# microsoft/rl-offline-simulation

Measured on AMD Instinct MI355X. Metric: simulated steps/sec (node), 10M logged transitions x 4096 rollouts, higher is better.
Workload: dtype f64

## Files before the change

### rl-offline-simulation_amd/csrc/offsim_hip.hip

```cpp
#include <hip/hip_fp16.h>
#include <hip/hip_runtime.h>
#include <mutex>
#include <stdint.h>
#include <stdio.h>
#include <stdlib.h>
#include <string.h>
#include <time.h>

#include "offsim.h"
#include "discount.hpp"
#include "pcg64_dev.hpp"
#include "philox_dev.hpp"
#include "stream_row.hpp"

extern "C" int offsim_lds_order_ok(void);
#include "shuffle_wave.hpp"
#include "shuffle_chunk.hpp"

using namespace offsim;

static thread_local char g_err[512] = "";

static int fail(int code, const char *fmt, const char *detail = "") {
    snprintf(g_err, sizeof(g_err), fmt, detail);
    return code;
}
#define HIP_TRY(expr)                                                        \
    do {                                                                     \
        hipError_t _e = (expr);                                              \
        if (_e != hipSuccess) return fail(OFFSIM_EHIP, #expr ": %s", hipGetErrorString(_e)); \
    } while (0)
#define LAUNCH_CHECK()                                                       \
    do {                                                                     \
        hipError_t _e = hipGetLastError();                                   \
        if (_e != hipSuccess) return fail(OFFSIM_EHIP, "kernel launch: %s", hipGetErrorString(_e)); \
    } while (0)

extern "C" const char *offsim_last_error(void) { return g_err; }
extern "C" int offsim_version(void) { return 100; }
extern "C" int offsim_device_count(void) {
    int n = 0;
    hipError_t e = hipGetDeviceCount(&n);
    if (e != hipSuccess) return fail(OFFSIM_EHIP, "hipGetDeviceCount: %s", hipGetErrorString(e));
    return n;
}


#define GRP_CHUNK 2048

__global__ void k_group_hist(const int32_t *__restrict__ slot, int64_t N, int32_t n_slots, uint32_t *__restrict__ hist) {
    extern __shared__ uint32_t lds_cnt[];
    for (int s = threadIdx.x; s < n_slots; s += blockDim.x) lds_cnt[s] = 0;
    __syncthreads();
    int64_t base = (int64_t)blockIdx.x * GRP_CHUNK;
    for (int i = threadIdx.x; i < GRP_CHUNK; i += blockDim.x) {
        int64_t row = base + i;
        if (row < N) atomicAdd(&lds_cnt[slot[row]], 1u);
    }
    __syncthreads();
    uint32_t *h = hist + (int64_t)blockIdx.x * n_slots;
    for (int s = threadIdx.x; s < n_slots; s += blockDim.x) h[s] = lds_cnt[s];
}

__global__ void k_group_scan_chunks(uint32_t *__restrict__ hist, int64_t n_chunks, int32_t n_slots, uint32_t *__restrict__ totals) {
    int s = blockIdx.x * blockDim.x + threadIdx.x;
    if (s >= n_slots) return;
    uint32_t run = 0;
    for (int64_t c = 0; c < n_chunks; c++) {
        uint32_t v = hist[c * n_slots + s];
        hist[c * n_slots + s] = run;
        run += v;
    }
    totals[s] = run;
}
__global__ void k_group_scan_slots(const uint32_t *__restrict__ totals, int32_t n_slots, uint32_t *__restrict__ seg_off) {
    uint32_t carry = 0;
    int lane = threadIdx.x;
    for (int b = 0; b < n_slots; b += WAVE) {
        int s = b + lane;
        uint32_t v = s < n_slots ? totals[s] : 0u;
        uint32_t inc = v;
#pragma unroll
        for (int d = 1; d < WAVE; d <<= 1) {
            uint32_t o = __shfl_up(inc, d);
            if (lane >= d) inc += o;
        }
        if (s < n_slots) seg_off[s] = carry + inc - v;
        carry += __shfl(inc, WAVE - 1);
    }
    if (lane == 0) seg_off[n_slots] = carry;
}
__global__ void k_group_scatter(const int32_t *__restrict__ slot, int64_t N, int32_t n_slots,
                                const uint32_t *__restrict__ hist, const uint32_t *__restrict__ seg_off,
                                int32_t *__restrict__ order) {
    extern __shared__ uint32_t lds_pos_raw[];
    volatile uint32_t *lds_pos = lds_pos_raw;
    const uint32_t *h = hist + (int64_t)blockIdx.x * n_slots;
    for (int s = threadIdx.x; s < n_slots; s += WAVE) lds_pos[s] = seg_off[s] + h[s];
    __syncthreads();
    int lane = threadIdx.x;
    int64_t base = (int64_t)blockIdx.x * GRP_CHUNK;
    for (int i = 0; i < GRP_CHUNK; i += WAVE) {
        int64_t row = base + i + lane;
        bool valid = row < N;
        int32_t key = valid ? slot[row] : -1;
        uint64_t todo = __ballot(valid);
        uint32_t dst = 0;
        while (todo) {
            int leader = __ffsll((unsigned long long)todo) - 1;
            int32_t k = __shfl(key, leader);
            uint64_t same = __ballot(valid && key == k);
            if (valid && key == k) {
                uint32_t before = __popcll(same & ((1ull << lane) - 1ull));
                dst = lds_pos[k] + before;
            }
            __builtin_amdgcn_s_waitcnt(0xc07f);
            if (lane == leader) lds_pos[k] += __popcll(same);
            todo &= ~same;
        }
        if (valid) order[dst] = (int32_t)row;
    }
}

extern "C" int64_t offsim_group_scratch_bytes(int64_t N, int32_t n_slots) {
    int64_t n_chunks = (N + GRP_CHUNK - 1) / GRP_CHUNK;
    if (n_chunks < 1) n_chunks = 1;
    return (n_chunks * n_slots + n_slots) * (int64_t)sizeof(uint32_t) + 256;
}

extern "C" int offsim_group_by_state(const int32_t *slot, int64_t N, int32_t n_slots, uint32_t *seg_off, int32_t *order,
                                     void *scratch, void *stream) {
    if (N < 0 || n_slots <= 0 || !seg_off || !scratch) return fail(OFFSIM_EINVAL, "group_by_state: bad argument%s");
    if ((int64_t)n_slots * 4 > 64 * 1024) return fail(OFFSIM_EUNSUPPORTED, "group_by_state: more than 16384 states%s");
    if (N >= (1ll << 31)) return fail(OFFSIM_EUNSUPPORTED, "group_by_state: N >= 2^31%s");
    hipStream_t st = (hipStream_t)stream;
    int64_t n_chunks = (N + GRP_CHUNK - 1) / GRP_CHUNK;
    uint32_t *hist = (uint32_t *)scratch;
    uint32_t *totals = hist + (n_chunks > 0 ? n_chunks : 1) * n_slots;
    if (n_chunks == 0) {
        HIP_TRY(hipMemsetAsync(seg_off, 0, sizeof(uint32_t) * (n_slots + 1), st));
        return OFFSIM_OK;
    }
    size_t lds = sizeof(uint32_t) * n_slots;
    hipLaunchKernelGGL(k_group_hist, dim3((unsigned)n_chunks), dim3(256), lds, st, slot, N, n_slots, hist);
    LAUNCH_CHECK();
    hipLaunchKernelGGL(k_group_scan_chunks, dim3((n_slots + 63) / 64), dim3(64), 0, st, hist, n_chunks, n_slots, totals);
    LAUNCH_CHECK();
    hipLaunchKernelGGL(k_group_scan_slots, dim3(1), dim3(WAVE), 0, st, totals, n_slots, seg_off);
    LAUNCH_CHECK();
    hipLaunchKernelGGL(k_group_scatter, dim3((unsigned)n_chunks), dim3(WAVE), lds, st, slot, N, n_slots, hist, seg_off, order);
    LAUNCH_CHECK();
    return OFFSIM_OK;
}

template <typename T>
__global__ void k_gather_elem(const T *__restrict__ src, const int32_t *__restrict__ order, int64_t N, T *__restrict__ dst) {
    int64_t g = (int64_t)blockIdx.x * blockDim.x + threadIdx.x;
    if (g < N) dst[g] = src[order[g]];
}
template <typename W>
__global__ void k_gather_words(const W *__restrict__ src, const int32_t *__restrict__ order, int64_t N, int32_t words, W *__restrict__ dst) {
    int64_t i = (int64_t)blockIdx.x * blockDim.x + threadIdx.x;
    if (i >= N * words) return;
    int64_t g = i / words;
    int32_t w = (int32_t)(i - g * words);
    dst[i] = src[(int64_t)order[g] * words + w];
}
extern "C" int offsim_gather_rows(const void *src, const int32_t *order, int64_t N, int32_t row_bytes, void *dst, void *stream) {
    if (N < 0 || row_bytes <= 0) return fail(OFFSIM_EINVAL, "gather_rows: bad argument%s");
    if (N == 0) return OFFSIM_OK;
    hipStream_t st = (hipStream_t)stream;
    unsigned nb = (unsigned)((N + 255) / 256);
    if (row_bytes == 1) hipLaunchKernelGGL(k_gather_elem<uint8_t>, dim3(nb), dim3(256), 0, st, (const uint8_t *)src, order, N, (uint8_t *)dst);
    else if (row_bytes == 2) hipLaunchKernelGGL(k_gather_elem<uint16_t>, dim3(nb), dim3(256), 0, st, (const uint16_t *)src, order, N, (uint16_t *)dst);
    else if (row_bytes == 4) hipLaunchKernelGGL(k_gather_elem<uint32_t>, dim3(nb), dim3(256), 0, st, (const uint32_t *)src, order, N, (uint32_t *)dst);
    else if (row_bytes == 8) hipLaunchKernelGGL(k_gather_elem<uint64_t>, dim3(nb), dim3(256), 0, st, (const uint64_t *)src, order, N, (uint64_t *)dst);
    else {
        const int32_t wb = row_bytes % 4 == 0 ? 4 : row_bytes % 2 == 0 ? 2 : 1, words = row_bytes / wb;
        unsigned nbw = (unsigned)((N * words + 255) / 256);
        if (wb == 4) hipLaunchKernelGGL(k_gather_words<uint32_t>, dim3(nbw), dim3(256), 0, st, (const uint32_t *)src, order, N, words, (uint32_t *)dst);
        else if (wb == 2) hipLaunchKernelGGL(k_gather_words<uint16_t>, dim3(nbw), dim3(256), 0, st, (const uint16_t *)src, order, N, words, (uint16_t *)dst);
        else hipLaunchKernelGGL(k_gather_words<uint8_t>, dim3(nbw), dim3(256), 0, st, (const uint8_t *)src, order, N, words, (uint8_t *)dst);
    }
    LAUNCH_CHECK();
    return OFFSIM_OK;
}

__global__ void k_seed_streams(const uint64_t *__restrict__ seeds, int32_t R, uint64_t *__restrict__ out) {
    int r = blockIdx.x * blockDim.x + threadIdx.x;
    if (r >= R) return;
    PcgInit p = pcg_seed(seeds[r]);
    out[4 * r + 0] = p.state.hi;
    out[4 * r + 1] = p.state.lo;
    out[4 * r + 2] = p.inc.hi;
    out[4 * r + 3] = p.inc.lo;
}
extern "C" int offsim_seed_streams(const uint64_t *seeds, int32_t R, uint64_t *rng_out, void *stream) {
    if (R < 0 || !seeds || !rng_out) return fail(OFFSIM_EINVAL, "seed_streams: bad argument%s");
    if (R == 0) return OFFSIM_OK;
    hipLaunchKernelGGL(k_seed_streams, dim3((R + 255) / 256), dim3(256), 0, (hipStream_t)stream, seeds, R, rng_out);
    LAUNCH_CHECK();
    return OFFSIM_OK;
}

__global__ void __launch_bounds__(64) k_pcg_jump_probe(const uint64_t *seeds, const uint32_t *counts, int32_t n_counts, int32_t halve,
                                                       uint64_t *out_tab, uint64_t *out_ref) {
    const uint32_t lane = threadIdx.x, g = blockIdx.x & 1u, ci = (blockIdx.x >> 1) % (uint32_t)n_counts, si = (blockIdx.x >> 1) / (uint32_t)n_counts;
    const PcgJumpRow lane_row = pcg_lane_row(64u * g + lane + 1u);
    const uint32_t q = sh_rfl(halve ? counts[ci] >> 1 : counts[ci]);
    const PcgInit p = pcg_seed(seeds[si]);
    const U128 st = pcg_chain_start(p, lane_row, q);
    const Jump j128 = pcg_jump_lane(p.inc, 128u);
    const U128 st_ref = pcg_apply(pcg_jump(p.inc, (uint64_t)q + 64ull * g + (uint64_t)lane + 1), p.state);
    const Jump j_ref = pcg_jump(p.inc, 128);
    uint64_t *ot = out_tab + (int64_t)blockIdx.x * OFFSIM_PCG_PROBE_WORDS, *orf = out_ref + (int64_t)blockIdx.x * OFFSIM_PCG_PROBE_WORDS;
    ot[2u * lane] = st.hi;
    ot[2u * lane + 1u] = st.lo;
    orf[2u * lane] = st_ref.hi;
    orf[2u * lane + 1u] = st_ref.lo;
    if (lane == 0) {
        ot[128] = j128.mult.hi, ot[129] = j128.mult.lo, ot[130] = j128.plus.hi, ot[131] = j128.plus.lo;
        orf[128] = j_ref.mult.hi, orf[129] = j_ref.mult.lo, orf[130] = j_ref.plus.hi, orf[131] = j_ref.plus.lo;
    }
}
extern "C" int offsim_pcg_jump_probe(const uint64_t *seeds, int32_t n_seeds, const uint32_t *counts, int32_t n_counts, int32_t halve,
                                     uint64_t *out_tab, uint64_t *out_ref, void *stream) {
    if (n_seeds < 0 || n_counts < 0 || !seeds || !counts || !out_tab || !out_ref) return fail(OFFSIM_EINVAL, "pcg_jump_probe: bad argument%s");
    if ((int64_t)n_seeds * n_counts > (1 << 20)) return fail(OFFSIM_EINVAL, "pcg_jump_probe: at most 2^20 {seed, count} pairs%s");
    if (n_seeds == 0 || n_counts == 0) return OFFSIM_OK;
    hipLaunchKernelGGL(k_pcg_jump_probe, dim3(2u * (unsigned)n_seeds * (unsigned)n_counts), dim3(64), 0, (hipStream_t)stream, seeds, counts, n_counts, halve,
                       out_tab, out_ref);
    LAUNCH_CHECK();
    return OFFSIM_OK;
}

static hipError_t allow_big_lds_fn(const void *fn, int bytes) {
    struct Seen {
        const void *fn;
        int max_bytes;
        uint64_t devs;
    };
    static thread_local Seen seen[64];
    static thread_local int n_seen = 0;
    int dev = 0;
    hipError_t e = hipGetDevice(&dev);
    if (e != hipSuccess) return e;
    Seen *hit = nullptr;
    for (int i = 0; i < n_seen; i++)
        if (seen[i].fn == fn) hit = &seen[i];
    if (hit && dev < 64 && bytes <= hit->max_bytes && ((hit->devs >> dev) & 1ull)) return hipSuccess;
    const int want = hit && hit->max_bytes > bytes ? hit->max_bytes : bytes;
    e = hipFuncSetAttribute(fn, hipFuncAttributeMaxDynamicSharedMemorySize, want);
    if (e != hipSuccess) return e;
    if (!hit && n_seen < 64) {
        hit = &seen[n_seen++];
        hit->fn = fn;
        hit->max_bytes = 0;
        hit->devs = 0;
    }
    if (hit) {
        if (want > hit->max_bytes) {
            hit->max_bytes = want;
            hit->devs = 0;
        }
        if (dev < 64) hit->devs |= 1ull << dev;
    }
    return hipSuccess;
}
#define allow_big_lds(kernel, bytes) allow_big_lds_fn((const void *)(kernel), (bytes))

template <int K>
static int shuf_launch_cuts(int n_launches, size_t lds_top, unsigned n_blocks, hipStream_t st, const offsim_table *t, const uint64_t *seeds, int32_t n_perm,
                            uint32_t *perm_out, uint32_t *init_perm_out, uint32_t lo, uint32_t hi, const uint32_t *dig32, uint32_t *dig_out,
                            uint16_t *loc_out, uint32_t a_xchg) {
    constexpr uint32_t TOP = K == 0 ? 0u : shuf_cuts[K > 0 ? K - 1 : 0], STOP = K == shuf_n_cuts ? 1u : shuf_cuts[K < shuf_n_cuts ? K : 0];
    constexpr uint32_t SQ = K == 0 ? SHUF_SQ_BIG : SHUF_SQ_SMALL;
    if (K >= n_launches) return OFFSIM_OK;
    const size_t ldsb = K == 0 ? lds_top : shuf_fixed_lds_bytes(SQ) + (size_t)TOP * 2 + 16;
    HIP_TRY(allow_big_lds((k_shuffle_wave<true, SQ, TOP, STOP>), 160 * 1024));
    hipLaunchKernelGGL((k_shuffle_wave<true, SQ, TOP, STOP>), dim3(n_blocks), dim3(256), ldsb, st, t->seg_off, t->n_slots, t->N, t->N0, seeds, n_perm,
                       perm_out, init_perm_out, lo, hi, dig32, dig_out, loc_out, a_xchg);
    LAUNCH_CHECK();
    if constexpr (K < shuf_n_cuts)
        return shuf_launch_cuts<K + 1>(n_launches, lds_top, n_blocks, st, t, seeds, n_perm, perm_out, init_perm_out, lo, hi, dig32, dig_out, loc_out, a_xchg);
    else
        return OFFSIM_OK;
}

static int lds_order_ok_on(void *stream);
static int launch_shuffle(const offsim_table *t, const uint64_t *seeds, int32_t n_perm, uint32_t *perm_out, uint32_t *init_perm_out,
                          const uint32_t *dig32, uint32_t *dig_out, uint16_t *loc_out, hipStream_t st, bool big_segments_elsewhere = false) {
    const uint32_t max_seg = t->max_seg > 0 ? (uint32_t)(t->max_seg > 0xffffffffll ? 0xffffffffll : t->max_seg) : 0xffffffffu;
    const uint32_t min_seg = t->min_seg > 0 ? (uint32_t)(t->min_seg > 0xffffffffll ? 0xffffffffll : t->min_seg) : 1u;
    const uint32_t n0 = (uint32_t)(t->N0 > 0xffffffffll ? 0xffffffffll : t->N0);
    const int64_t n_blocks = (int64_t)(t->n_slots + 1) * n_perm;
    if (n_blocks > 0x7fffffffll) return fail(OFFSIM_EUNSUPPORTED, "shuffle_queues: too many chains%s");
    HIP_TRY(allow_big_lds((k_shuffle_wave<true, SHUF_SQ_BIG>), 160 * 1024));
    HIP_TRY(allow_big_lds((k_shuffle_wave<true, SHUF_SQ_SMALL>), 160 * 1024));
    static const bool no_xchg = getenv("OFFSIM_SHUFFLE_XCHG") && atoi(getenv("OFFSIM_SHUFFLE_XCHG")) == 0;
    const int okv = lds_order_ok_on(st);
    if (okv < 0) return okv;
    const uint32_t a_xchg = (okv == 1 && !no_xchg) ? 1u : 0u;
    if (!big_segments_elsewhere && (max_seg > SHUF_CAP16 || n0 > SHUF_CAP16)) {
        hipLaunchKernelGGL((k_shuffle_wave<false, SHUF_SQ_SMALL>), dim3((unsigned)n_blocks), dim3(256), shuf_fixed_lds_bytes(SHUF_SQ_SMALL), st, t->seg_off,
                           t->n_slots, t->N, t->N0, seeds, n_perm, perm_out, init_perm_out, SHUF_CAP16, 0xffffffffu, dig32, dig_out, loc_out, 0u);
        LAUNCH_CHECK();
    }
    static const uint32_t bounds[] = {SHUF_CAP16, 32768u, 8192u, 2048u, 0u};
    for (int k = 0; k < 4; k++) {
        const uint32_t hi = bounds[k], lo = bounds[k + 1];
        const bool seg_in = min_seg <= hi && max_seg > lo, init_in = n0 > lo && n0 <= hi;
        if (!seg_in && !init_in) continue;
        uint32_t need = 0;
        if (seg_in) need = max_seg < hi ? max_seg : hi;
        if (init_in && n0 > need) need = n0;
        const uint32_t sq = k == 0 ? SHUF_SQ_BIG : SHUF_SQ_SMALL;
        const size_t lds16 = shuf_fixed_lds_bytes(sq) + (((size_t)need * 2 + 15) & ~(size_t)15) + 16;
        if (k == 0 && dig_out) {
#ifdef SHUF_PROF
            const int prof_launches = getenv("OFFSIM_SHUFFLE_PROF_LAUNCHES") ? atoi(getenv("OFFSIM_SHUFFLE_PROF_LAUNCHES")) : shuf_n_cuts + 1;
#else
            const int prof_launches = shuf_n_cuts + 1;
#endif
            const int rc = shuf_launch_cuts<0>(prof_launches, lds16, (unsigned)n_blocks, st, t, seeds, n_perm, perm_out, init_perm_out, lo, hi, dig32, dig_out,
                                               loc_out, a_xchg);
            if (rc != OFFSIM_OK) return rc;
            if (init_in)
                hipLaunchKernelGGL((k_shuffle_wave<true, SHUF_SQ_BIG>), dim3((unsigned)n_perm), dim3(256), lds16, st, t->seg_off, t->n_slots, t->N,
                                   t->N0, seeds, n_perm, perm_out, init_perm_out, lo, hi, dig32, nullptr, nullptr, a_xchg);
        } else if (k == 0)
            hipLaunchKernelGGL((k_shuffle_wave<true, SHUF_SQ_BIG>), dim3((unsigned)n_blocks), dim3(256), lds16, st, t->seg_off, t->n_slots, t->N, t->N0,
                               seeds, n_perm, perm_out, init_perm_out, lo, hi, dig32, dig_out, loc_out, a_xchg);
        else
            hipLaunchKernelGGL((k_shuffle_wave<true, SHUF_SQ_SMALL>), dim3((unsigned)n_blocks), dim3(256), lds16, st, t->seg_off, t->n_slots, t->N, t->N0,
                               seeds, n_perm, perm_out, init_perm_out, lo, hi, dig32, dig_out, loc_out, a_xchg);
        LAUNCH_CHECK();
    }
    return OFFSIM_OK;
}

__global__ void k_fault_exchange(int32_t *out) { *out = atomicExch(&offsim::g_async_fault, 0); }

extern "C" int offsim_async_faults(void) {
    static int32_t *slot[64] = {nullptr};
    static std::mutex mu;
    std::lock_guard<std::mutex> hold(mu);
    int dev = 0;
    if (hipGetDevice(&dev) != hipSuccess || dev < 0 || dev >= 64) return fail(OFFSIM_EHIP, "async_faults: no device%s");
    if (!slot[dev] && hipMalloc((void **)&slot[dev], sizeof(int32_t)) != hipSuccess) return fail(OFFSIM_EHIP, "async_faults: allocation failed%s");
    hipLaunchKernelGGL(k_fault_exchange, dim3(1), dim3(1), 0, (hipStream_t)0, slot[dev]);
    if (hipGetLastError() != hipSuccess) return fail(OFFSIM_EHIP, "async_faults: launch failed%s");
    int32_t v = 0;
    if (hipMemcpy(&v, slot[dev], sizeof(v), hipMemcpyDeviceToHost) != hipSuccess) return fail(OFFSIM_EHIP, "async_faults: read failed%s");
    return v;
}

extern "C" int offsim_shuffle_queues(const offsim_table *t, const uint64_t *seeds, int32_t n_perm, uint32_t *perm_out,
                                     uint32_t *init_perm_out, void *stream) {
    if (!t || !seeds || n_perm < 0 || !perm_out || !init_perm_out) return fail(OFFSIM_EINVAL, "shuffle_queues: bad argument%s");
    if (n_perm == 0) return OFFSIM_OK;
    return launch_shuffle(t, seeds, n_perm, perm_out, init_perm_out, nullptr, nullptr, nullptr, (hipStream_t)stream);
}

__global__ void __launch_bounds__(256) k_big_keys(const uint32_t *__restrict__ seg_off, int64_t N, const uint32_t *__restrict__ dig32,
                                                  uint32_t *__restrict__ dig_out, uint16_t *__restrict__ loc_out, uint32_t r0) {
    const uint32_t s = blockIdx.y, r = r0 + blockIdx.z;
    const uint32_t beg = seg_off[s], len = seg_off[s + 1] - beg;
    if (len <= SHUF_CAP16) return;
    for (uint32_t k = blockIdx.x * 1024u + threadIdx.x; k < len && k < (blockIdx.x + 1u) * 1024u; k += 256u) {
        const int64_t p = (int64_t)r * N + beg + k;
        const uint32_t row = dig_out[p], loc = row - beg, h = loc >> 16;
        dig_out[p] = dig32[row] | ((h & 3u) << 8) | ((h >> 2) << 11);
        loc_out[p] = (uint16_t)loc;
    }
}

#define SHC_HEADER_BYTES 4096
static uint32_t shc_cb() {
    static const int v = getenv("OFFSIM_SHUFFLE_CHUNK") ? atoi(getenv("OFFSIM_SHUFFLE_CHUNK")) : 0;
    return v == 16384 ? 16384u : v == 8192 ? 8192u : v == 2048 ? 2048u : 4096u;
}
static uint32_t shc_longest(const offsim_table *t) {
    const int64_t a = t->max_seg > (int64_t)SHUF_CAP16 ? t->max_seg : 0, b = t->N0 > (int64_t)SHUF_CAP16 ? t->N0 : 0;
    return (uint32_t)(a > b ? a : b);
}
static int64_t shc_block_words(const offsim_table *t, uint32_t *msg_cap_out, int64_t *lc_words_out = nullptr, bool plain = false) {
    const uint32_t n = shc_longest(t), cb = shc_cb();
    const uint64_t msg = shc_pool_entries(n, cb), rep = (uint64_t)((n + cb - 1u) / cb) * cb;
    if (msg_cap_out) *msg_cap_out = (uint32_t)msg;
    if (lc_words_out) *lc_words_out = plain ? 0 : (int64_t)((n + 3u) / 4u);
    if (plain) return (int64_t)(msg + rep);
    return (int64_t)(msg + (msg + 1u) / 2u + rep + (n + 3u) / 4u);
}
extern "C" int64_t offsim_shuffle_workspace_bytes(const offsim_table *t, int32_t n_blocks) {
    if (!t || n_blocks < 1 || shc_longest(t) == 0 || t->max_seg > (1ll << 23) || t->N0 > (1ll << 23)) return 0;
    return SHC_HEADER_BYTES + (int64_t)n_blocks * shc_block_words(t, nullptr) * 8;
}

struct ShcPlan {
    int64_t n_wg = 0, words = 0, lc_words = 0;
    uint32_t msg_cap = 0, kcap = 0, lds_b = 0;
};
static ShcPlan shc_plan(const offsim_table *t, void *workspace, int64_t workspace_bytes, bool plain) {
    ShcPlan p;
    if (shc_longest(t) == 0 || t->max_seg > (1ll << 23) || t->N0 > (1ll << 23) || !workspace || ((uintptr_t)workspace & 7u) != 0) return p;
    if (t->n_slots + 1 > (SHC_HEADER_BYTES / 4 - 64)) return p;
    p.words = shc_block_words(t, &p.msg_cap, &p.lc_words, plain);
    p.n_wg = (workspace_bytes - SHC_HEADER_BYTES) / (p.words * 8);
    int dev = 0, cus = 256;
    if (hipGetDevice(&dev) == hipSuccess) (void)hipDeviceGetAttribute(&cus, hipDeviceAttributeMultiprocessorCount, dev);
    p.kcap = (shc_longest(t) + shc_cb() - 1u) / shc_cb();
#define SHC_LDSB(PL)                                                                                                                    \
    (shc_cb() == 16384u ? shc_lds_bytes<16384u, 2048u, 1024u, PL>(p.kcap) : shc_cb() == 4096u ? shc_lds_bytes<4096u, 1024u, 512u, PL>(p.kcap) \
     : shc_cb() == 2048u ? shc_lds_bytes<2048u, 1024u, 512u, PL>(p.kcap) : shc_lds_bytes<8192u, 1024u, 512u, PL>(p.kcap))
    p.lds_b = plain ? SHC_LDSB(true) : SHC_LDSB(false);
#undef SHC_LDSB
    const int64_t per_cu = (160 * 1024) / (int64_t)((p.lds_b + 1023u) & ~1023u);
    p.n_wg = p.n_wg > cus * per_cu ? cus * per_cu : p.n_wg;
    if (p.n_wg < 1) p.n_wg = 0;
    return p;
}
static int shc_launch(const ShcPlan &p, const offsim_table *t, const uint64_t *seeds, int32_t n_perm, const uint32_t *dig32, uint32_t *dig_out,
                      void *loc_out, uint32_t *init_perm_out, uint32_t *perm_out, void *workspace, hipStream_t st, uint32_t loc_bits = 16u,
                      uint32_t chains_above = SHUF_CAP16) {
    { const int okv = lds_order_ok_on(st); if (okv < 0) return okv; if (okv == 0) return fail(OFFSIM_EUNSUPPORTED, "chunked shuffle: this device's LDS does not serve same-address lanes of one instruction in lane order (offsim_lds_order_ok): lend no workspace -- the in-place shuffle does not need it%s"); }
    uint32_t *hdr = (uint32_t *)workspace;
    hipLaunchKernelGGL(k_chunk_worklist, dim3(1), dim3(256), 0, st, t->seg_off, t->n_slots, (uint32_t)(t->N0 > 0xffffffffll ? 0xffffffffll : t->N0), chains_above,
                       hdr + 64, hdr + 1, hdr);
    LAUNCH_CHECK();
#define SHC_LAUNCH_(CB, RG, SQ, PL)                                                                                                     \
    do {                                                                                                                                \
        HIP_TRY(allow_big_lds((k_shuffle_chunked<CB, RG, SQ, PL>), 160 * 1024));                                                         \
        hipLaunchKernelGGL((k_shuffle_chunked<CB, RG, SQ, PL>), dim3((unsigned)p.n_wg), dim3(256), p.lds_b, st, t->seg_off, t->N, seeds, n_perm,  \
                           hdr + 64, hdr + 1, hdr, (uint64_t *)((char *)workspace + SHC_HEADER_BYTES), p.words, p.msg_cap, p.kcap, dig32,   \
                           dig_out, loc_out, t->n_slots, t->N0, init_perm_out, perm_out, p.lc_words, loc_bits);                         \
    } while (0)
#define SHC_LAUNCH(CB, RG, SQ)                                                                                                          \
    do {                                                                                                                                \
        if (perm_out) SHC_LAUNCH_(CB, RG, SQ, true);                                                                                    \
        else SHC_LAUNCH_(CB, RG, SQ, false);                                                                                            \
    } while (0)
    if (shc_cb() == 16384u) SHC_LAUNCH(16384u, 2048u, 1024u);
    else if (shc_cb() == 4096u) SHC_LAUNCH(4096u, 1024u, 512u);
    else if (shc_cb() == 2048u) SHC_LAUNCH(2048u, 1024u, 512u);
    else SHC_LAUNCH(8192u, 1024u, 512u);
#undef SHC_LAUNCH
#undef SHC_LAUNCH_
    LAUNCH_CHECK();
    return OFFSIM_OK;
}

extern "C" int offsim_shuffle_queues_ws(const offsim_table *t, const uint64_t *seeds, int32_t n_perm, uint32_t *perm_out, uint32_t *init_perm_out,
                                        void *workspace, int64_t workspace_bytes, void *stream) {
    if (!t || !seeds || n_perm < 0 || !perm_out || !init_perm_out) return fail(OFFSIM_EINVAL, "shuffle_queues: bad argument%s");
    if (n_perm == 0) return OFFSIM_OK;
    const ShcPlan p = t->max_seg > 0 ? shc_plan(t, workspace, workspace_bytes, true) : ShcPlan();
    int rc = launch_shuffle(t, seeds, n_perm, perm_out, init_perm_out, nullptr, nullptr, nullptr, (hipStream_t)stream, p.n_wg >= 1);
    if (rc || p.n_wg < 1) return rc;
    return shc_launch(p, t, seeds, n_perm, nullptr, nullptr, nullptr, init_perm_out, perm_out, workspace, (hipStream_t)stream);
}

extern "C" int offsim_shuffle_queues_keys_ws(const offsim_table *t, const uint64_t *seeds, int32_t n_perm, const uint32_t *dig32, int32_t format,
                                             uint32_t *dig_out, void *loc_out, uint32_t *init_perm_out, void *workspace, int64_t workspace_bytes,
                                             void *stream) {
    if (!t || !seeds || n_perm < 0 || !init_perm_out || (t->N > 0 && (!dig32 || !dig_out || !loc_out)))
        return fail(OFFSIM_EINVAL, "shuffle_queues_keys: bad argument%s");
    if (format != OFFSIM_STREAMS_A && format != OFFSIM_STREAMS_B && format != OFFSIM_STREAMS_C) return fail(OFFSIM_EINVAL, "shuffle_queues_keys: bad format%s");
    if (t->max_seg <= 0 && t->N > 0) return fail(OFFSIM_EINVAL, "shuffle_queues_keys: offsim_table.max_seg must be set%s");
    const bool big = t->max_seg > (int64_t)SHUF_CAP16;
    if (format == OFFSIM_STREAMS_C) {
        if (t->max_seg > (1ll << 17) || t->n_slots > 255 || t->N0 > (1ll << 23))
            return fail(OFFSIM_EUNSUPPORTED, "shuffle_queues_keys: format C holds 2^17 rows per state, 255 states%s");
        if (n_perm == 0 || t->N == 0) return OFFSIM_OK;
        offsim_table tc = *t;
        if (tc.max_seg <= (int64_t)SHUF_CAP16) tc.max_seg = (int64_t)SHUF_CAP16 + 1;
        const ShcPlan pc = shc_plan(&tc, workspace, workspace_bytes, false);
        if (pc.n_wg < 1) return fail(OFFSIM_EUNSUPPORTED, "shuffle_queues_keys: format C needs a workspace (offsim_shuffle_workspace_bytes)%s");
        return shc_launch(pc, &tc, seeds, n_perm, dig32, dig_out, loc_out, init_perm_out, nullptr, workspace, (hipStream_t)stream, 8u, 0u);
    }
    if (big && format != OFFSIM_STREAMS_B)
        return fail(OFFSIM_EUNSUPPORTED, "shuffle_queues_keys: a state has more than 65536 rows: stream format B (or offsim_shuffle_queues)%s");
    if (big && (t->max_seg > (1ll << 23) || t->n_slots > 255)) return fail(OFFSIM_EUNSUPPORTED, "shuffle_queues_keys: format B holds 2^23 rows per state, 255 states%s");
    if (n_perm == 0) return OFFSIM_OK;
    hipStream_t st = (hipStream_t)stream;
    const ShcPlan p = shc_plan(t, workspace, workspace_bytes, false);
    const bool chunked = p.n_wg >= 1;
    int rc = launch_shuffle(t, seeds, n_perm, big && !chunked ? dig_out : nullptr, init_perm_out, dig32, dig_out, (uint16_t *)loc_out, st, chunked);
    if (rc || (!big && !chunked)) return rc;
    if (chunked) return shc_launch(p, t, seeds, n_perm, dig32, dig_out, loc_out, init_perm_out, nullptr, workspace, st);
    for (int32_t r0 = 0; r0 < n_perm; r0 += 65535) {
        const int32_t nz = n_perm - r0 < 65535 ? n_perm - r0 : 65535;
        hipLaunchKernelGGL(k_big_keys, dim3((unsigned)((t->max_seg + 1023) / 1024), (unsigned)t->n_slots, (unsigned)nz), dim3(256), 0, st,
                           t->seg_off, t->N, dig32, dig_out, (uint16_t *)loc_out, (uint32_t)r0);
        LAUNCH_CHECK();
    }
    return OFFSIM_OK;
}

extern "C" int offsim_shuffle_queues_keys(const offsim_table *t, const uint64_t *seeds, int32_t n_perm, const uint32_t *dig32, int32_t format,
                                          uint32_t *dig_out, void *loc_out, uint32_t *init_perm_out, void *stream) {
    return offsim_shuffle_queues_keys_ws(t, seeds, n_perm, dig32, format, dig_out, loc_out, init_perm_out, nullptr, 0, stream);
}

__global__ void k_env_reset(offsim_table t, offsim_rollouts ro, const uint8_t *__restrict__ mask, int32_t *__restrict__ out_row) {
    int r = blockIdx.x * blockDim.x + threadIdx.x;
    if (r >= ro.R) return;
    if (mask && !mask[r]) return;
    uint32_t ic = ro.init_cursor[r];
    if ((int64_t)ic >= t.N0) {
        ro.cur_slot[r] = -1;
        if (out_row) out_row[r] = -1;
        return;
    }
    uint32_t k = ro.init_perm ? ro.init_perm[(int64_t)r * ro.init_stride + ic] : ic;
    ro.init_cursor[r] = ic + 1;
    ro.cur_slot[r] = t.init_slot[k];
    if (out_row) out_row[r] = t.init_orig[k];
}
extern "C" int offsim_env_reset(const offsim_table *t, offsim_rollouts *ro, const uint8_t *mask, int32_t *out_init_row,
                                void *stream) {
    if (!t || !ro || ro->R < 0) return fail(OFFSIM_EINVAL, "env_reset: bad argument%s");
    if (ro->R == 0) return OFFSIM_OK;
    hipLaunchKernelGGL(k_env_reset, dim3((ro->R + 255) / 256), dim3(256), 0, (hipStream_t)stream, *t, *ro, mask, out_init_row);
    LAUNCH_CHECK();
    return OFFSIM_OK;
}
__global__ void k_env_set_state(offsim_rollouts ro, const int32_t *__restrict__ slot, const uint8_t *__restrict__ mask) {
    int r = blockIdx.x * blockDim.x + threadIdx.x;
    if (r >= ro.R) return;
    if (mask && !mask[r]) return;
    ro.cur_slot[r] = slot[r];
}
struct VecCols {
    offsim_column c[8];
};
__global__ void k_vector_gather(const int32_t *__restrict__ row, const int32_t *__restrict__ status, const uint8_t *__restrict__ mask, int32_t R,
                                VecCols cols, int32_t n_cols, uint8_t *__restrict__ alive) {
    const int k = blockIdx.x * blockDim.x + threadIdx.x;
    if (k >= R) return;
    const int32_t rw = row[k];
    bool ok;
    if (status) {
        ok = status[k] == OFFSIM_ST_OK && rw >= 0;
        if (alive) alive[k] = (uint8_t)(alive[k] && ok);
    } else {
        const bool m = mask ? mask[k] != 0 : true;
        ok = m && rw >= 0;
        if (alive && m) alive[k] = (uint8_t)(rw >= 0);
    }
    for (int c = 0; c < n_cols; c++) {
        const int64_t nb = cols.c[c].row_bytes;
        unsigned char *d = (unsigned char *)cols.c[c].dst + (int64_t)k * nb;
        if (ok) {
            const unsigned char *sp = (const unsigned char *)cols.c[c].src + (int64_t)rw * nb;
            if (((nb | (int64_t)(uintptr_t)sp | (int64_t)(uintptr_t)d) & 3) == 0) {
                for (int64_t b = 0; b < nb; b += 4) *(uint32_t *)(d + b) = *(const uint32_t *)(sp + b);
            } else {
                for (int64_t b = 0; b < nb; b++) d[b] = sp[b];
            }
        } else if (cols.c[c].zero_if_not_ok) {
            for (int64_t b = 0; b < nb; b++) d[b] = 0;
        }
    }
}

extern "C" int offsim_vector_gather(const int32_t *row, const int32_t *status, const uint8_t *mask, int32_t R, const offsim_column *cols,
                                    int32_t n_cols, uint8_t *alive, void *stream) {
    if (!row || R < 0 || n_cols < 0 || n_cols > 8 || (n_cols > 0 && !cols)) return fail(OFFSIM_EINVAL, "vector_gather: bad argument%s");
    VecCols vc;
    memset(&vc, 0, sizeof(vc));
    for (int c = 0; c < n_cols; c++) {
        if (!cols[c].src || !cols[c].dst || cols[c].row_bytes <= 0) return fail(OFFSIM_EINVAL, "vector_gather: bad column%s");
        vc.c[c] = cols[c];
    }
    if (R == 0) return OFFSIM_OK;
    hipLaunchKernelGGL(k_vector_gather, dim3((unsigned)((R + 255) / 256)), dim3(256), 0, (hipStream_t)stream, row, status, mask, R, vc, n_cols,
                       alive);
    LAUNCH_CHECK();
    return OFFSIM_OK;
}
// ... 1643 lines not shown
```

Baseline: 16.51 billion.

## Add single-wave kernel for the low shuffle stage of segment permutation

Adds k_shuffle_low, a 64-thread single-wavefront kernel that finishes the final (lowest) cut of the per-segment Fisher-Yates shuffle. Each wave batches PCG draws, accepts swaps with ballots, detects conflicts between lanes and applies swaps in conflict-free pieces in LDS, then gathers the digests and writes them out. It replaces the 256-thread k_shuffle_wave launch for the last cut unless OFFSIM_SHUFFLE_LOW=0. The aim is to drop block-level synchronisation and shrink LDS so more blocks stay resident, at the cost of a more intricate conflict-resolution path that must stay equivalent to the original permutation.

```diff
diff --git a/rl-offline-simulation_amd/csrc/offsim_hip.hip b/rl-offline-simulation_amd/csrc/offsim_hip.hip
--- a/rl-offline-simulation_amd/csrc/offsim_hip.hip
+++ b/rl-offline-simulation_amd/csrc/offsim_hip.hip
@@ -15,6 +15,7 @@
 
 extern "C" int offsim_lds_order_ok(void);
 #include "shuffle_wave.hpp"
+#include "shuffle_low.hpp"
 #include "shuffle_chunk.hpp"
 
 using namespace offsim;
@@ -276,6 +277,15 @@
     constexpr uint32_t TOP = K == 0 ? 0u : shuf_cuts[K > 0 ? K - 1 : 0], STOP = K == shuf_n_cuts ? 1u : shuf_cuts[K < shuf_n_cuts ? K : 0];
     constexpr uint32_t SQ = K == 0 ? SHUF_SQ_BIG : SHUF_SQ_SMALL;
     if (K >= n_launches) return OFFSIM_OK;
+    if constexpr (K == shuf_n_cuts && K > 0) {
+        static const bool no_low = getenv("OFFSIM_SHUFFLE_LOW") && atoi(getenv("OFFSIM_SHUFFLE_LOW")) == 0;
+        if (!no_low) {
+            hipLaunchKernelGGL((k_shuffle_low<TOP>), dim3(n_blocks), dim3(64), shuf_low_lds_bytes(TOP), st, t->seg_off, t->n_slots, t->N, seeds, n_perm, lo, hi,
+                               dig32, dig_out, loc_out, a_xchg);
+            LAUNCH_CHECK();
+            return OFFSIM_OK;
+        }
+    }
     const size_t ldsb = K == 0 ? lds_top : shuf_fixed_lds_bytes(SQ) + (size_t)TOP * 2 + 16;
     HIP_TRY(allow_big_lds((k_shuffle_wave<true, SQ, TOP, STOP>), 160 * 1024));
     hipLaunchKernelGGL((k_shuffle_wave<true, SQ, TOP, STOP>), dim3(n_blocks), dim3(256), ldsb, st, t->seg_off, t->n_slots, t->N, t->N0, seeds, n_perm,
diff --git a/rl-offline-simulation_amd/csrc/shuffle_low.hpp b/rl-offline-simulation_amd/csrc/shuffle_low.hpp
--- /dev/null
+++ b/rl-offline-simulation_amd/csrc/shuffle_low.hpp
@@ -0,0 +1,264 @@
+#pragma once
+#include "shuffle_wave.hpp"
+
+namespace offsim {
+
+#define SHUF_LOW_RG 256u
+#define SHUF_LOW_SQ 256u
+#ifndef SHUF_LOW_W
+#define SHUF_LOW_W 64u
+#endif
+static_assert(SHUF_LOW_W == 64u || SHUF_LOW_W == 32u || SHUF_LOW_W == 16u, "SHUF_LOW_W: 64, 32 or 16 steps per group");
+constexpr uint32_t shuf_low_lds_bytes(uint32_t top) { return 2u * top + 2u * SHUF_LOW_RG + 2u * SHUF_LOW_SQ; }
+
+template <uint32_t TOP, class MID>
+__device__ __forceinline__ void shuf_low_fill(lds_vu16 *x16, const uint16_t *lc, uint32_t lane, MID mid) {
+    typedef uint32_t u32x4_a4 __attribute__((ext_vector_type(4), aligned(4)));
+    typedef uint32_t u32x4 __attribute__((ext_vector_type(4)));
+    constexpr uint32_t VEC = TOP / 8u, PER = VEC / 64u, RJ = PER < 4u ? PER : 4u;
+    static_assert(TOP >= 1024u && (TOP & (TOP - 1u)) == 0u, "a cut: a power of two, 1024 at least");
+    const bool odd = (((uintptr_t)lc >> 1) & 1u) != 0u;
+    const uint32_t *src = (const uint32_t *)(lc - (odd ? 1 : 0));
+    __attribute__((address_space(3))) u32x4 *dst = (__attribute__((address_space(3))) u32x4 *)x16;
+#pragma unroll 1
+    for (uint32_t r0 = 0; r0 < PER; r0 += RJ) {
+        u32x4 w[RJ];
+        uint32_t e[RJ];
+#pragma unroll
+        for (uint32_t j = 0; j < RJ; j++) {
+            const uint32_t q = lane + 64u * (r0 + j);
+            w[j] = *(const u32x4_a4 *)(src + 4u * q);
+            e[j] = odd ? src[4u * q + 4u] : 0u;
+        }
+        __builtin_amdgcn_sched_barrier(0);
+        if (r0 == 0u) mid();
+        __builtin_amdgcn_sched_barrier(0);
+#pragma unroll
+        for (uint32_t j = 0; j < RJ; j++) {
+            const uint32_t q = lane + 64u * (r0 + j);
+            u32x4 o = w[j];
+            if (odd) {
+                o.x = __builtin_amdgcn_alignbyte(w[j].y, w[j].x, 2u);
+                o.y = __builtin_amdgcn_alignbyte(w[j].z, w[j].y, 2u);
+                o.z = __builtin_amdgcn_alignbyte(w[j].w, w[j].z, 2u);
+                o.w = __builtin_amdgcn_alignbyte(e[j], w[j].w, 2u);
+            }
+            dst[q] = o;
+        }
+    }
+}
+
+template <uint32_t TOP>
+__global__ void __launch_bounds__(64)
+    k_shuffle_low(const uint32_t *__restrict__ seg_off, int32_t n_slots, int64_t N, const uint64_t *__restrict__ seeds, int32_t n_perm, uint32_t n_lo,
+                  uint32_t n_hi, const uint32_t *__restrict__ dig32, uint32_t *__restrict__ dig_out, uint16_t *__restrict__ loc_out, uint32_t a_xchg) {
+    extern __shared__ __align__(16) unsigned char lds_raw[];
+    lds_vu16 *x16 = (lds_vu16 *)lds_raw;
+    lds_vu16 *dr = x16 + TOP;
+    lds_vu32 *drw = (lds_vu32 *)dr;
+    lds_vu16 *jq = dr + SHUF_LOW_RG;
+    static_assert(TOP <= 32768u, "draws and partners are kept in 16 bits");
+#ifdef SHUF_PROF
+    const uint64_t pf_entry = __builtin_amdgcn_s_memtime();
+#endif
+    const uint32_t lane = threadIdx.x;
+
+    const int32_t s_idx = (int32_t)(blockIdx.x / (uint32_t)n_perm);
+    const int32_t r = (int32_t)(blockIdx.x - (uint32_t)s_idx * (uint32_t)n_perm);
+    if (s_idx == 0 || s_idx > n_slots || dig_out == nullptr) return;
+    const uint32_t base_val = seg_off[s_idx - 1];
+    const uint32_t n_rows = seg_off[s_idx] - base_val;
+    if (n_rows <= n_lo || n_rows > n_hi || n_rows <= TOP) return;
+    const uint32_t *dsrc = dig32 + base_val;
+    uint32_t *dg = dig_out + (int64_t)r * N + base_val;
+    uint16_t *lc = loc_out + (int64_t)r * N + base_val;
+
+    const PcgJumpRow lane_row = pcg_lane_row(lane + 1u);
+    uint32_t c_start = 0;
+    U128 st = u128(0, 0);
+    Jump j64;
+    j64.mult = j64.plus = u128(0, 0);
+    shuf_low_fill<TOP>(x16, lc, lane, [&]() __attribute__((always_inline)) {
+        c_start = sh_rfl(dg[0]);
+        const PcgInit p = pcg_seed(seeds[r]);
+        j64 = pcg_jump_lane(p.inc, 64u);
+        st = pcg_chain_start(p, lane_row, c_start >> 1);
+    });
+
+#ifdef SHUF_PROF
+    uint64_t pf_gen = 0, pf_cls = 0, pf_app = 0, pf_cut = 0, pf_t = 0;
+    const uint64_t pf_begin = __builtin_amdgcn_s_memtime();
+#define SLP0() pf_t = __builtin_amdgcn_s_memtime()
+#define SLP1(acc) acc += __builtin_amdgcn_s_memtime() - pf_t
+#else
+#define SLP0()
+#define SLP1(acc)
+#endif
+    typedef __attribute__((address_space(3))) unsigned char lds_b8;
+    const uint32_t x16_a = (uint32_t)(uintptr_t)(lds_b8 *)x16;
+
+    uint32_t i_top = TOP - 1u, done = 0, fill = 0;
+    auto apply = [&](const uint32_t cnt) __attribute__((always_inline)) {
+        const uint32_t i_first = i_top, il = i_first - lane, lo_g = i_first - cnt;
+        const bool in = lane < cnt;
+        const uint32_t v = in ? (uint32_t)jq[(done + lane) & (SHUF_LOW_SQ - 1u)] : 0u;
+        done += cnt;
+        i_top -= cnt;
+        uint64_t confl = __ballot(in && v < il && v > lo_g), cuts = 0;
+#ifdef SHUF_PROF
+        const bool had = confl != 0ull;
+        if (had) SLP0();
+#endif
+        while (confl) {
+            cuts |= 1ull << (i_first - sh_rfl((uint32_t)__builtin_amdgcn_readlane((int)v, (int)sh_ff1(confl))));
+            confl &= confl - 1ull;
+        }
+        if (a_xchg) {
+            const uint32_t pid = in ? (uint32_t)sh_rank(cuts) + (uint32_t)((cuts >> lane) & 1ull) : 0xffffffffu;
+            const uint32_t first = (uint32_t)(cuts & 1ull), n_pieces = (uint32_t)__popcll(cuts & ~1ull) + 1u;
+            const uint32_t sh = (v & 1u) << 4, ad = x16_a + ((v & ~1u) << 1);
+            for (uint32_t pc = first; pc < first + n_pieces; pc++) {
+                if (pid == pc) {
+                    const uint32_t a = (uint32_t)x16[il];
+                    uint32_t old;
+                    asm volatile("ds_mskor_rtn_b32 %0, %1, %2, %3\n\ts_waitcnt lgkmcnt(0)" : "=v"(old) : "v"(ad), "v"(0xffffu << sh), "v"(a << sh) : "memory");
+                    x16[il] = (uint16_t)(old >> sh);
+                }
+            }
+        } else {
+            uint32_t tg = lane;
+            if (in) {
+                const uint32_t b = (uint32_t)x16[v];
+                x16[v] = (uint16_t)lane;
+                tg = (uint32_t)x16[v];
+                x16[v] = (uint16_t)b;
+            }
+            uint64_t F = __ballot(tg != lane);
+            if (F) {
+                uint64_t D = F;
+                while (F) {
+                    D |= 1ull << sh_rfl((uint32_t)__builtin_amdgcn_readlane((int)tg, (int)sh_ff1(F)));
+                    F &= F - 1ull;
+                }
+                cuts |= D & (D - 1ull);
+            }
+            const uint32_t pid = in ? (uint32_t)sh_rank(cuts) + (uint32_t)((cuts >> lane) & 1ull) : 0xffffffffu;
+            const uint32_t first = (uint32_t)(cuts & 1ull), n_pieces = (uint32_t)__popcll(cuts & ~1ull) + 1u;
+            for (uint32_t pc = first; pc < first + n_pieces; pc++) {
+                if (pid == pc) {
+                    const uint32_t a2 = (uint32_t)x16[il], b2 = (uint32_t)x16[v];
+                    x16[il] = (uint16_t)b2;
+                    x16[v] = (uint16_t)a2;
+                }
+            }
+        }
+#ifdef SHUF_PROF
+        if (had) SLP1(pf_cut);
+#endif
+    };
+
+    uint32_t i = TOP - 1u, c = c_start & 1u, avail = 0, blk = 0;
+    uint32_t mask = 0xffffffffu >> __builtin_clz(i);
+    int lowpow = (int)((mask >> 1) + 1u);
+    auto settle = [&](uint64_t &bal, int &rk, uint32_t v, uint32_t ib) {
+        uint64_t f = bal & __ballot((int)v > (int)ib - rk);
+        while (f) {
+            bal &= ~(1ull << sh_ff1(f));
+            rk = sh_rank(bal);
+            f = bal & __ballot((int)v > (int)ib - rk);
+        }
+    };
+    while (i >= 1u) {
+        if (avail < c + 64u) {
+            SLP0();
+            const uint64_t o = pcg_output(st);
+            st = pcg_apply(j64, st);
+            drw[((blk & 1u) << 6) + lane] = ((uint32_t)o & 0xffffu) | ((uint32_t)(o >> 32) << 16);
+            blk++;
+            avail += 128u;
+            SLP1(pf_gen);
+        }
+        SLP0();
+        const uint32_t v = (uint32_t)dr[(c + lane) & (SHUF_LOW_RG - 1u)] & mask;
+        uint64_t bal = __ballot(v <= i);
+        int rk = sh_rank(bal);
+        settle(bal, rk, v, i);
+        uint32_t na = (uint32_t)__popcll(bal);
+        if (__builtin_expect((int)i - (int)na >= lowpow, 1)) {
+            c += 64u;
+        } else {
+            const uint64_t lowm = __ballot((int)i - rk < lowpow);
+            const uint64_t below = (lowm & (0ull - lowm)) - 1ull;
+            bal &= below;
+            na = (uint32_t)__popcll(bal);
+            c += (uint32_t)__popcll(below);
+        }
+        if ((bal >> lane) & 1ull) jq[(fill + (uint32_t)rk) & (SHUF_LOW_SQ - 1u)] = (uint16_t)v;
+        fill += na;
+        i -= na;
+        if ((int)i < lowpow && i >= 1u) {
+            mask = 0xffffffffu >> __builtin_clz(i);
+            lowpow = (int)((mask >> 1) + 1u);
+        }
+        SLP1(pf_cls);
+        SLP0();
+        while (fill - done >= SHUF_LOW_W) apply(SHUF_LOW_W);
+        SLP1(pf_app);
+    }
+    if (fill != done) {
+        SLP0();
+        apply(fill - done);
+        SLP1(pf_app);
+    }
+#ifdef SHUF_PROF
+    const uint64_t pf_end = __builtin_amdgcn_s_memtime();
+#endif
+
+    {
+        lds_vu32 *xw = (lds_vu32 *)x16;
+        const bool lc_dword = (((uintptr_t)lc >> 1) & 1u) == 0u;
+#pragma unroll 1
+        for (uint32_t k0 = lane; k0 < TOP / 2u; k0 += 256u) {
+            uint32_t two[4], d0[4], d1[4];
+#pragma unroll
+            for (int u = 0; u < 4; u++) two[u] = xw[k0 + 64u * (uint32_t)u];
+#pragma unroll
+            for (int u = 0; u < 4; u++) {
+                const uint32_t i0 = two[u] & 0xffffu, i1 = two[u] >> 16;
+                d0[u] = dsrc[i0 < n_rows ? i0 : 0u];
+                d1[u] = dsrc[i1 < n_rows ? i1 : 0u];
+            }
+#pragma unroll
+            for (int u = 0; u < 4; u++) {
+                const uint32_t k = k0 + 64u * (uint32_t)u;
+                dg[2u * k] = d0[u];
+                dg[2u * k + 1u] = d1[u];
+                if (lc_dword) {
+                    *(uint32_t *)(lc + 2u * k) = two[u];
+                } else {
+                    lc[2u * k] = (uint16_t)(two[u] & 0xffffu);
+                    lc[2u * k + 1u] = (uint16_t)(two[u] >> 16);
+                }
+            }
+        }
+    }
+#ifdef SHUF_PROF
+    __builtin_amdgcn_s_waitcnt(0);
+    if (lane == 0) {
+        const uint64_t now = __builtin_amdgcn_s_memtime();
+        for (int w = 0; w < 12; w++) dg[w] = 0u;
+        dg[0] = (uint32_t)(pf_gen >> 6);
+        dg[3] = (uint32_t)(pf_cls >> 6);
+        dg[6] = (uint32_t)(pf_app >> 6);
+        dg[8] = (uint32_t)(pf_cut >> 6);
+        dg[12] = (uint32_t)((now - pf_begin) >> 6);
+        dg[13] = (uint32_t)((pf_begin - pf_entry) >> 6);
+        dg[14] = (uint32_t)((now - pf_end) >> 6);
+        dg[15] = 0u;
+    }
+#endif
+#undef SLP0
+#undef SLP1
+}
+
+}
```

Result: no change. 16.66 billion, median of 6 (+0.9%).
